# aaletov/open-pcc-metric

Measured on AMD Instinct MI355X. Metric: Mpoints/s for symmetric D1+D2 PSNR, N_ref=N_deg=1M, higher is better.
Workload: dtype f64

## Files before the change

open_pcc_metric_amd/csrc/pccm_api.hip:

```cpp
#include <cxxabi.h>
#include <dlfcn.h>
#include <math.h>
#include <stdarg.h>
#include <stdio.h>
#include <string.h>

#include <chrono>
#include <new>
#include <thread>

#include "pccm_stale.h"

namespace pccm {

static thread_local char g_err[512] = "";

int fail(int code, const char *fmt, ...)
{
    va_list ap;
    va_start(ap, fmt);
    vsnprintf(g_err, sizeof(g_err), fmt, ap);
    va_end(ap);
    return code;
}

int ensure(pccm_ctx *ctx, DevBuf &b, size_t bytes)
{
    if (bytes <= b.bytes && b.p) return PCCM_OK;
    if (ctx->capturing) {
        ctx->capture_failed = true;
        return fail(PCCM_E_STATE, "a buffer must grow during graph capture: run the same call sequence once before capturing");
    }
    ctx->epoch++;
    if (b.p) {
        PCCM_HIP(hipStreamSynchronize(ctx->stream));
        PCCM_HIP(hipFree(b.p));
        b.p = nullptr;
        b.bytes = 0;
    }
    size_t want = bytes < 256 ? 256 : bytes;
    PCCM_HIP(hipMalloc(&b.p, want));
    b.bytes = want;
    return PCCM_OK;
}

int grow(void **p, size_t &cap, size_t bytes)
{
    if (*p && cap >= bytes) return PCCM_OK;
    if (*p) {
        (void)hipFree(*p);
        *p = nullptr;
        cap = 0;
    }
    PCCM_HIP(hipMalloc(p, bytes ? bytes : 1));
    cap = bytes;
    return PCCM_OK;
}

int check_device_errors(pccm_ctx *ctx)
{
    if (!ctx->host_err) return PCCM_OK;
    const uint32_t e = __atomic_exchange_n(ctx->host_err, 0u, __ATOMIC_RELAXED);
    if (!e) return PCCM_OK;
    results_dropped(ctx);
    return fail(PCCM_E_STATE, "a search kernel reported an inconsistent state (device error word 0x%x: %s%s%s): the results of this search were "
                              "dropped, run it again", e, (e & 1u) ? "the tail launch's wait for its own workgroups ran out; " : "",
                (e & 2u) ? "a voxel brick contradicts its cell start; " : "", (e & kErrMergeTable) ? "the duplicate table overflowed" : "");
}

static hipEvent_t take_event(pccm_ctx *ctx)
{
    if (!ctx->event_pool.empty()) {
        hipEvent_t e = ctx->event_pool.back();
        ctx->event_pool.pop_back();
        return e;
    }
    hipEvent_t e = nullptr;
    if (hipEventCreate(&e) != hipSuccess) return nullptr;
    return e;
}

ProfScope::ProfScope(pccm_ctx *c, int k) : ctx(c), cls(k)
{
    if (!ctx->prof_on || ctx->capturing) return;
    a = take_event(ctx);
    b = take_event(ctx);
    if (a) (void)hipEventRecord(a, ctx->stream);
}

ProfScope::~ProfScope()
{
    if (!ctx->prof_on || ctx->capturing || !a || !b) return;
    (void)hipEventRecord(b, ctx->stream);
    ctx->spans.push_back({a, b, cls});
}

static int collect_spans(pccm_ctx *ctx)
{
    if (ctx->spans.empty()) return PCCM_OK;
    PCCM_HIP(hipStreamSynchronize(ctx->stream));
    for (auto &s : ctx->spans) {
        float ms = 0.f;
        if (hipEventElapsedTime(&ms, s.a, s.b) == hipSuccess) {
            ctx->prof_ms[s.cls] += ms;
            ctx->prof_n[s.cls] += 1;
        }
        ctx->event_pool.push_back(s.a);
        ctx->event_pool.push_back(s.b);
    }
    ctx->spans.clear();
    return PCCM_OK;
}

static void free_buf(DevBuf &b)
{
    if (b.p) (void)hipFree(b.p);
    b.p = nullptr;
    b.bytes = 0;
}

// ... 9 lines not shown
}

static void free_nn(NNResult &r)
{
    free_buf(r.flagged);
    free_buf(r.flag_thr);
    free_buf(r.tail);
    free_buf(r.rec);
    r.form = NNForm{};
    if (r.idx) (void)hipFree(r.idx);
    if (r.d2) (void)hipFree(r.d2);
    r.idx = nullptr;
    r.d2 = nullptr;
    r.cap = 0;
}

static void shard_of(int64_t n, int rank, int world, int64_t *b, int64_t *e)
{
    if (world <= 0) {
        *b = 0;
        *e = 0;
        return;
    }
    const int64_t unit = n >= (int64_t)world * kChunk ? kChunk : kLeaf;
    const int64_t units = (n + unit - 1) / unit;
    int64_t u0 = units * rank / world, u1 = units * (rank + 1) / world;
    int64_t lo = u0 * unit, hi = u1 * unit;
    *b = lo < n ? lo : n;
    *e = hi < n ? hi : n;
}

static int dir_clouds(pccm_ctx *ctx, int dir, const Cloud **it, const Cloud **se)
{
    if (dir == PCCM_DIR_LEFT) { *it = &ctx->cloud[0]; *se = &ctx->cloud[1]; }
    else if (dir == PCCM_DIR_RIGHT) { *it = &ctx->cloud[1]; *se = &ctx->cloud[0]; }
    else if (dir == PCCM_DIR_SELF) { *it = &ctx->cloud[0]; *se = &ctx->cloud[0]; }
    else return fail(PCCM_E_ARG, "bad direction %d", dir);
    if ((*it)->n <= 0 || (*se)->n <= 0) return fail(PCCM_E_STATE, "clouds are not set");
    return PCCM_OK;
}

static void host_copy(void *dst, const void *src, size_t bytes)
{
    constexpr size_t kPiece = 1u << 20;
    const int nt = bytes >= 8 * kPiece ? 4 : bytes >= 2 * kPiece ? 2 : 1;
    if (nt == 1) {
        memcpy(dst, src, bytes);
        return;
    }
    std::thread th[3];
    const size_t part = (bytes / nt + 63) & ~(size_t)63;
    for (int k = 1; k < nt; ++k) {
        const size_t off = (size_t)k * part, len = k + 1 < nt ? part : bytes - off;
        th[k - 1] = std::thread([=] { memcpy((char *)dst + off, (const char *)src + off, len); });
    }
    memcpy(dst, src, part);
    for (int k = 1; k < nt; ++k) th[k - 1].join();
}

static int pin_ensure(pccm_ctx *ctx, int which, size_t bytes)
{
    if (ctx->pin_cap[which] >= bytes) return PCCM_OK;
    if (ctx->pin[which]) {
        PCCM_HIP(hipDeviceSynchronize());
        (void)hipHostFree(ctx->pin[which]);
        ctx->pin[which] = nullptr;
        ctx->pin_cap[which] = 0;
    }
    const size_t cap = (bytes + (bytes >> 2) + 4095) & ~(size_t)4095;
    if (hipHostMalloc(&ctx->pin[which], cap, hipHostMallocDefault) != hipSuccess) {
        (void)hipGetLastError();
        ctx->pin[which] = nullptr;
        return fail(PCCM_E_OOM, "hipHostMalloc of %zu bytes (transfer staging) failed", cap);
    }
    ctx->pin_cap[which] = cap;
    return PCCM_OK;
}

constexpr size_t kStagedFrom = 32u << 10;
constexpr size_t kPinWindow = 64u << 20;

static int h2d(pccm_ctx *ctx, void *dev, const void *host, size_t bytes, hipStream_t st)
{
    if (!ctx->io_staged || bytes < kStagedFrom) {
        PCCM_HIP(hipMemcpyAsync(dev, host, bytes, hipMemcpyHostToDevice, st));
        return PCCM_OK;
    }
    const int which = st == ctx->stream ? 0 : 1;
    if (!ctx->pin_ev[which]) PCCM_HIP(hipEventCreateWithFlags(&ctx->pin_ev[which], hipEventDisableTiming));
    if (ctx->pin_ev_set[which]) PCCM_HIP(hipEventSynchronize(ctx->pin_ev[which]));
    int rc = pin_ensure(ctx, which, bytes < kPinWindow ? bytes : kPinWindow);
    if (rc) return rc;
    constexpr size_t kChunk = 4u << 20;
    static_assert(kPinWindow % kChunk == 0, "whole pieces per window");
    for (size_t off = 0; off < bytes; off += kChunk) {
        const size_t len = bytes - off < kChunk ? bytes - off : kChunk, at = off % kPinWindow;
        if (off && at == 0) {
            PCCM_HIP(hipEventRecord(ctx->pin_ev[which], st));
            PCCM_HIP(hipEventSynchronize(ctx->pin_ev[which]));
        }
        host_copy((char *)ctx->pin[which] + at, (const char *)host + off, len);
        PCCM_HIP(hipMemcpyAsync((char *)dev + off, (char *)ctx->pin[which] + at, len, hipMemcpyHostToDevice, st));
    }
    PCCM_HIP(hipEventRecord(ctx->pin_ev[which], st));
    ctx->pin_ev_set[which] = true;
    return PCCM_OK;
}

static int d2h(pccm_ctx *ctx, void *host, const void *dev, size_t bytes)
{
// ... 2365 lines not shown
```

open_pcc_metric_amd/csrc/pccm_gridbuild.hip:

```cpp
#include "pccm_grid.h"

namespace pccm {

constexpr int kLbItems = 64;
constexpr int kLbTile = 256 * kLbItems;

int64_t scan_tiles(int64_t m) { return (m + kLbTile - 1) / kLbTile; }

__global__ __launch_bounds__(256) void k_scan_lookback(uint32_t *__restrict__ data, int64_t m, unsigned long long *__restrict__ state,
                                                       int64_t ntiles)
{
    __shared__ uint32_t s_tile, s_prefix, wsum[4];
    const int tid = threadIdx.x, lane = tid & 63, w = tid >> 6;
    if (tid == 0) s_tile = (uint32_t)atomicAdd(&state[ntiles], 1ull);
    __syncthreads();
    const int64_t tile = s_tile;
    const int64_t base = tile * kLbTile + (int64_t)tid * kLbItems;
    uint32_t v[kLbItems], tot = 0;
    if (base + kLbItems <= m) {
#pragma unroll
        for (int k = 0; k < kLbItems; k += 4) {
            const uint4 q = *reinterpret_cast<const uint4 *>(&data[base + k]);
            v[k] = q.x; v[k + 1] = q.y; v[k + 2] = q.z; v[k + 3] = q.w;
        }
    } else {
#pragma unroll
        for (int k = 0; k < kLbItems; ++k) v[k] = (base + k < m) ? data[base + k] : 0u;
    }
#pragma unroll
    for (int k = 0; k < kLbItems; ++k) tot += v[k];
    uint32_t inc = tot;
#pragma unroll
    for (int off = 1; off < 64; off <<= 1) {
        const uint32_t o = __shfl_up(inc, off);
        if (lane >= off) inc += o;
    }
    if (lane == 63) wsum[w] = inc;
    __syncthreads();
    uint32_t woff = 0;
    for (int k = 0; k < w; ++k) woff += wsum[k];
    const uint32_t agg = wsum[0] + wsum[1] + wsum[2] + wsum[3];
    if (w == 0) {
        if (lane == 0)
            __hip_atomic_store(&state[tile], ((tile == 0 ? 2ull : 1ull) << 32) | agg, __ATOMIC_RELAXED, __HIP_MEMORY_SCOPE_AGENT);
        uint32_t excl = 0;
        int64_t p = tile - 1;
        while (p >= 0) {
            const int64_t idx = p - lane;
            const unsigned long long st = idx >= 0 ? __hip_atomic_load(&state[idx], __ATOMIC_RELAXED, __HIP_MEMORY_SCOPE_AGENT)
                                                   : (2ull << 32);
            const uint32_t status = (uint32_t)(st >> 32), val = (uint32_t)st;
            const unsigned long long incl = __ballot(status == 2u), empty = __ballot(status == 0u);
            const int first = incl ? __ffsll((long long)incl) - 1 : 64;
            const unsigned long long nearer = first >= 64 ? ~0ull : ((1ull << first) - 1ull);
            if (empty & nearer) {
                __builtin_amdgcn_s_sleep(2);
                continue;
            }
            uint32_t part = (lane <= first) ? val : 0u;
#pragma unroll
            for (int off = 32; off > 0; off >>= 1) part += __shfl_xor(part, off);
            excl += part;
            if (first < 64) break;
            p -= 64;
        }
        if (lane == 0) {
            if (tile > 0) __hip_atomic_store(&state[tile], (2ull << 32) | (unsigned long long)(excl + agg), __ATOMIC_RELAXED,
                                             __HIP_MEMORY_SCOPE_AGENT);
            s_prefix = excl;
        }
    }
    __syncthreads();
    uint32_t run = s_prefix + woff + inc - tot;
    if (base + kLbItems <= m) {
#pragma unroll
        for (int k = 0; k < kLbItems; k += 4) {
            uint4 q;
            q.x = run; run += v[k];
            q.y = run; run += v[k + 1];
            q.z = run; run += v[k + 2];
            q.w = run; run += v[k + 3];
            *reinterpret_cast<uint4 *>(&data[base + k]) = q;
        }
    } else {
#pragma unroll
        for (int k = 0; k < kLbItems; ++k) {
            if (base + k < m) data[base + k] = run;
            run += v[k];
        }
    }
}

constexpr int kRegK = 8;
constexpr int kRegRecs = 256 * kRegK;
constexpr int kMaxLg = 13;

struct BinJob {
    const double *x64;
    const float *x32;
    int64_t row0, n;
    uint32_t *cs;
    int64_t tl;
    int64_t nt;
    int64_t hoff;
    int64_t base;
    int64_t tile0;
    const float4 *sp;
    uint32_t *occ;
};

__device__ __forceinline__ void write_cell_starts(const BinJob &J, const uint32_t *s_cnt, int64_t c0, int nc, uint32_t first, uint32_t m)
{
    const int tid = threadIdx.x, nth = (int)blockDim.x;
    if (!J.occ) {
        for (int c = tid; c < nc; c += nth) J.cs[c0 + c] = first + s_cnt[c];
        return;
    }
    for (int c = tid; c < ((nc + 63) & ~63); c += nth) {
        const uint32_t here = c < nc ? s_cnt[c] : m, next = c + 1 < nc ? s_cnt[c + 1] : m;
        if (c < nc) J.cs[c0 + c] = first + here;
        const unsigned long long bits = __ballot(next != here);
        if ((tid & 63) == 0) {
            J.occ[(c0 + c) >> 5] = (uint32_t)bits;
            J.occ[((c0 + c) >> 5) + 1] = (uint32_t)(bits >> 32);
        }
    }
}

struct BinPlan {
    BinJob j[2];
    int njobs;
    int lg;
    int nbin;
    int64_t ncells;
    int64_t ntiles;
    int64_t hlen;
    int64_t state_off;
    int64_t nstate;
    uint32_t *zero;
    int nzero;
    uint32_t *cursor, *toff, *bstart;
};

template <bool X32>
__device__ __forceinline__ void load_point(const BinJob &J, int64_t i, double &x, double &y, double &z)
{
    const int64_t r = J.row0 + i;
    if (X32) {
        const float *q = J.x32 + (r >> 2) * 12 + (r & 3);
        x = (double)q[0];
        y = (double)q[4];
        z = (double)q[8];
    } else {
        const double *p = J.x64 + 3 * r;
        x = p[0];
        y = p[1];
        z = p[2];
    }
}

__device__ __forceinline__ void load_quad(const BinJob &J, int64_t i, float4 &x, float4 &y, float4 &z)
{
    const float4 *q = reinterpret_cast<const float4 *>(J.x32 + ((J.row0 + i) >> 2) * 12);
    x = q[0];
    y = q[1];
    z = q[2];
}

__device__ __forceinline__ int tile_job(const BinPlan &P, int64_t &tile)
{
    if (P.njobs > 1 && tile >= P.j[0].nt) {
        tile -= P.j[0].nt;
        return 1;
    }
    return 0;
}

template <bool X32, bool CUR>
__global__ __launch_bounds__(1024) void k_bin_count(BinPlan P, GridGeom g, uint32_t *__restrict__ hist)
{
    extern __shared__ uint32_t s_hist[];
    const int tid = threadIdx.x, nth = (int)blockDim.x;
    if (!CUR && blockIdx.x == 0) {
        unsigned long long *state = reinterpret_cast<unsigned long long *>(hist + P.state_off);
        if (tid == 0) hist[P.hlen] = 0u;
        for (int64_t k = tid; k < P.nstate; k += nth) state[k] = 0ull;
    }
    for (int b = tid; b < P.nbin; b += nth) s_hist[b] = 0u;
    __syncthreads();
    int64_t tile = blockIdx.x;
    const int jb = tile_job(P, tile);
    const BinJob &J = P.j[jb];
    const int64_t i0 = tile * J.tl, i1 = (i0 + J.tl < J.n) ? i0 + J.tl : J.n;
    if (X32 && J.sp) {
// ... 16 lines not shown
            for (int u = 0; u < 2; ++u) {
                const int64_t q = qd + (int64_t)u * nth;
                load_quad(J, i0 + 4 * (q < nquad ? q : nquad - 1), x[u], y[u], z[u]);
            }
#pragma unroll
            for (int u = 0; u < 2; ++u) {
                const int64_t i = i0 + 4 * (qd + (int64_t)u * nth);
                const float xs[4] = {x[u].x, x[u].y, x[u].z, x[u].w}, ys[4] = {y[u].x, y[u].y, y[u].z, y[u].w},
                            zs[4] = {z[u].x, z[u].y, z[u].z, z[u].w};
#pragma unroll
                for (int k = 0; k < 4; ++k)
                    if (i + k < i1) atomicAdd(&s_hist[cell_linear(g, (double)xs[k], (double)ys[k], (double)zs[k]) >> P.lg], 1u);
            }
        }
    } else {
        for (int64_t i = i0 + tid; i < i1; i += 4 * nth) {
            uint32_t bin[4];
#pragma unroll
            for (int k = 0; k < 4; ++k) {
                const int64_t ii = i + nth * k;
                double x, y, z;
                load_point<X32>(J, ii < i1 ? ii : i1 - 1, x, y, z);
                bin[k] = cell_linear(g, x, y, z) >> P.lg;
            }
#pragma unroll
            for (int k = 0; k < 4; ++k)
                if (i + nth * k < i1) atomicAdd(&s_hist[bin[k]], 1u);
        }
    }
    __syncthreads();
    if (CUR) {
        uint32_t *cur = P.cursor + (int64_t)jb * P.nbin, *dst = P.toff + (J.tile0 + tile) * P.nbin;
        for (int b = tid; b < P.nbin; b += nth) {
            const uint32_t c = s_hist[b];
            dst[b] = c ? atomicAdd(&cur[b], c) : 0u;
        }
        return;
    }
    uint32_t *dst = hist + J.hoff + tile;
    for (int b = tid; b < P.nbin; b += nth) dst[(int64_t)b * J.nt] = s_hist[b];
}

__device__ __forceinline__ void block_scan_inplace(uint32_t *s_cnt, int nc, uint32_t *s_wsum, uint32_t *s_carry);

template <typename REC, bool X32, bool CUR>
__global__ __launch_bounds__(1024) void k_bin_scatter(BinPlan P, GridGeom g, const uint32_t *__restrict__ hist, REC *__restrict__ tmp)
{
    extern __shared__ uint32_t s_cur[];
    __shared__ uint32_t s_wsum[16], s_carry;
    const int tid = threadIdx.x, nth = (int)blockDim.x;
    int64_t tile = blockIdx.x;
    const int jb = tile_job(P, tile);
    const BinJob &J = P.j[jb];
    if (CUR) {
        const uint32_t *tot = P.cursor + (int64_t)jb * P.nbin, *off = P.toff + (J.tile0 + tile) * P.nbin;
        uint32_t mine[2];
#pragma unroll
        for (int k = 0; k < 2; ++k) mine[k] = (tid + nth * k < P.nbin) ? off[tid + nth * k] : 0u;
        for (int b = tid; b < P.nbin; b += nth) s_cur[b] = tot[b];
        __syncthreads();
        block_scan_inplace(s_cur, P.nbin, s_wsum, &s_carry);
        if (tile == 0) {
            uint32_t *bs = P.bstart + (int64_t)jb * P.nbin;
            for (int b = tid; b < P.nbin; b += nth) bs[b] = (uint32_t)J.base + s_cur[b];
        }
        if (blockIdx.x == 0) {
            const BinJob &L = P.j[P.njobs - 1];
            if (tid == 0) P.bstart[(int64_t)P.njobs * P.nbin] = (uint32_t)(L.base + L.n);
            for (int k = 0; k < P.njobs; ++k)
                if (P.j[k].nt == 0)
                    for (int b = tid; b < P.nbin; b += nth) P.bstart[(int64_t)k * P.nbin + b] = (uint32_t)P.j[k].base;
        }
        __syncthreads();
#pragma unroll
        for (int k = 0; k < 2; ++k)
            if (tid + nth * k < P.nbin) s_cur[tid + nth * k] += (uint32_t)J.base + mine[k];
        for (int b = tid + 2 * nth; b < P.nbin; b += nth) s_cur[b] += (uint32_t)J.base + off[b];
    } else {
        const uint32_t *src = hist + J.hoff + tile;
        for (int b = tid; b < P.nbin; b += nth) s_cur[b] = src[(int64_t)b * J.nt];
    }
    __syncthreads();
    const int64_t i0 = tile * J.tl, i1 = (i0 + J.tl < J.n) ? i0 + J.tl : J.n;
    if (X32 && J.sp) {
        float4 *__restrict__ out = reinterpret_cast<float4 *>(tmp);
        for (int64_t i = i0 + tid; i < i1; i += 8 * nth) {
            float4 r[8];
#pragma unroll
            for (int k = 0; k < 8; ++k) {
                const int64_t ii = i + (int64_t)nth * k;
                r[k] = J.sp[J.row0 + (ii < i1 ? ii : i1 - 1)];
            }
#pragma unroll
            for (int k = 0; k < 8; ++k)
                if (i + (int64_t)nth * k < i1) {
                    const uint32_t pos = atomicAdd(&s_cur[cell_linear(g, (double)r[k].x, (double)r[k].y, (double)r[k].z) >> P.lg], 1u);
                    if (sizeof(REC) == 16) out[pos] = r[k];
                }
        }
        return;
    }
    if (X32) {
        const int64_t nquad = (i1 - i0 + 3) >> 2;
        for (int64_t qd = tid; qd < nquad; qd += 2 * nth) {
            float4 x[2], y[2], z[2];
#pragma unroll
// ... 39 lines not shown
}

__device__ __forceinline__ void block_scan_inplace(uint32_t *s_cnt, int nc, uint32_t *s_wsum, uint32_t *s_carry)
{
    const int tid = threadIdx.x, lane = tid & 63, w = tid >> 6;
    if (tid == 0) *s_carry = 0u;
    __syncthreads();
    const int nth = (int)blockDim.x;
    for (int base = 0; base < nc; base += 4 * nth) {
        const int e = base + 4 * tid;
        uint32_t c0 = e < nc ? s_cnt[e] : 0u, c1 = e + 1 < nc ? s_cnt[e + 1] : 0u;
        uint32_t c2 = e + 2 < nc ? s_cnt[e + 2] : 0u, c3 = e + 3 < nc ? s_cnt[e + 3] : 0u;
        const uint32_t tot = c0 + c1 + c2 + c3;
        uint32_t inc = tot;
#pragma unroll
        for (int off = 1; off < 64; off <<= 1) {
            const uint32_t o = __shfl_up(inc, off);
            if (lane >= off) inc += o;
        }
        if (lane == 63) s_wsum[w] = inc;
        __syncthreads();
        uint32_t run = *s_carry + inc - tot;
        for (int k = 0; k < w; ++k) run += s_wsum[k];
        if (e < nc) s_cnt[e] = run;
        run += c0;
        if (e + 1 < nc) s_cnt[e + 1] = run;
        run += c1;
        if (e + 2 < nc) s_cnt[e + 2] = run;
        run += c2;
        if (e + 3 < nc) s_cnt[e + 3] = run;
        __syncthreads();
        if (tid == nth - 1) *s_carry = run + c3;
        __syncthreads();
    }
}

__device__ __forceinline__ uint32_t rec_cell(const GridGeom &g, const float4 &r) { return cell_linear(g, (double)r.x, (double)r.y, (double)r.z); }
__device__ __forceinline__ uint32_t rec_cell(const GridGeom &g, const double4 &r) { return cell_linear(g, r.x, r.y, r.z); }
template <typename REC> struct RawRec;
template <> struct RawRec<Rec32> { typedef float4 type; };
template <> struct RawRec<GridRec> { typedef double4 type; };

template <typename REC>
__global__ __launch_bounds__(256, sizeof(REC) == 16 ? 6 : 4) void k_bin_sort(BinPlan P, GridGeom g, const uint32_t *__restrict__ hist, const REC *__restrict__ tmp,
                                                  REC *__restrict__ recs)
{
    extern __shared__ uint32_t s_cnt[];
    __shared__ uint32_t s_wsum[16], s_carry;
    const int tid = threadIdx.x;
    const int jb = (P.njobs > 1 && (int)blockIdx.x >= P.nbin) ? 1 : 0;
    const int b = (int)blockIdx.x - jb * P.nbin;
    const BinJob &J = P.j[jb];
    uint32_t s, e, j0;
    if (P.cursor) {
        const uint32_t *bs = P.bstart + (int64_t)jb * P.nbin + b;
        s = bs[0];
        e = bs[1];
        j0 = (uint32_t)J.base;
        if (tid == 0) P.cursor[(int64_t)jb * P.nbin + b] = 0u;
    } else {
        s = hist[J.hoff + (int64_t)b * J.nt];
        e = hist[J.hoff + (int64_t)(b + 1) * J.nt];
        j0 = hist[J.hoff];
    }
    const uint32_t m = e - s;
    const int64_t c0 = (int64_t)b << P.lg;
    const int nc = (int)((c0 + (1ll << P.lg) < P.ncells ? c0 + (1ll << P.lg) : P.ncells) - c0);
    for (int c = tid; c < nc; c += 256) s_cnt[c] = 0u;
    __syncthreads();
    if (m <= (uint32_t)kRegRecs) {
        typedef typename RawRec<REC>::type RAW;
        const RAW *__restrict__ src = reinterpret_cast<const RAW *>(tmp);
        RAW *__restrict__ dst = reinterpret_cast<RAW *>(recs);
        RAW v[kRegK];
        uint32_t cell[kRegK], rank[kRegK];
#pragma unroll
        for (int k = 0; k < kRegK; ++k) {
            const uint32_t i = tid + 256u * k;
            if (i < m) v[k] = src[s + i];
        }
#pragma unroll
        for (int k = 0; k < kRegK; ++k)
            if (tid + 256u * k < m) {
                cell[k] = rec_cell(g, v[k]) - (uint32_t)c0;
                rank[k] = atomicAdd(&s_cnt[cell[k]], 1u);
            }
        __syncthreads();
        block_scan_inplace(s_cnt, nc, s_wsum, &s_carry);
        write_cell_starts(J, s_cnt, c0, nc, s - j0, m);
#pragma unroll
        for (int k = 0; k < kRegK; ++k)
            if (tid + 256u * k < m) dst[s + s_cnt[cell[k]] + rank[k]] = v[k];
    } else {
        for (uint32_t i = tid; i < m; i += 256) {
            const P3 v = load_rec(tmp, s + i);
            atomicAdd(&s_cnt[cell_linear(g, v.x, v.y, v.z) - (uint32_t)c0], 1u);
        }
        __syncthreads();
        block_scan_inplace(s_cnt, nc, s_wsum, &s_carry);
        write_cell_starts(J, s_cnt, c0, nc, s - j0, m);
        __syncthreads();
        for (uint32_t i = tid; i < m; i += 256) {
            const P3 v = load_rec(tmp, s + i);
            const uint32_t pos = atomicAdd(&s_cnt[cell_linear(g, v.x, v.y, v.z) - (uint32_t)c0], 1u);
            store_rec(recs, s + pos, v);
        }
    }
    if (b == P.nbin - 1 && tid == 0) J.cs[P.ncells] = e - j0;
    if (blockIdx.x == 0 && tid < P.nzero) P.zero[tid] = 0u;
}

static int ceil_log2(int64_t v)
{
    int l = 0;
    while ((1ll << l) < v) ++l;
    return l;
}

int sort_by_cell(pccm_ctx *ctx, const BuildJobs &jobs, const GridGeom &g, int64_t ncells, void *recs, bool rec32, uint32_t *zero, int nzero)
{
    BinPlan P;
    P.zero = zero;
    P.nzero = zero ? nzero : 0;
    P.njobs = jobs.njobs;
    P.ncells = ncells;
    int lg = ceil_log2((ncells + 8191) / 8192);
    P.lg = lg < 10 ? 10 : (lg > kMaxLg ? kMaxLg : lg);
    {
        int64_t nmax = 0;
        for (int k = 0; k < jobs.njobs; ++k) nmax = jobs.j[k].n > nmax ? jobs.j[k].n : nmax;
        while (P.lg > 6 && (double)nmax * (double)(1ll << P.lg) / (double)ncells > 2000.0 && ((ncells >> (P.lg - 1)) + 1) <= 8192) --P.lg;
    }
    static const int lg_env = [] { const char *e = PCCM_DIAG_ENV("PCCM_BUILD_LG"); return e ? atoi(e) : 0; }();
    if (lg_env >= 8 && lg_env <= kMaxLg && (ncells >> lg_env) < 8192) P.lg = lg_env;
    P.nbin = (int)((ncells + (1ll << P.lg) - 1) >> P.lg);
    if (P.nbin > 8192) return fail(PCCM_E_ARG, "grid of %lld cells is too large", (long long)ncells);
    P.ntiles = 0;
    for (int k = 0; k < 2; ++k) {
        const BuildJob &s = jobs.j[k < jobs.njobs ? k : 0];
        BinJob &d = P.j[k];
        d.x64 = s.x64; d.x32 = s.x32; d.row0 = s.row0; d.cs = s.cs;
        d.sp = rec32 ? reinterpret_cast<const float4 *>(s.sp) : nullptr;
        d.occ = s.occ;
        if (rec32 && k < jobs.njobs && (s.row0 & 3)) return fail(PCCM_E_ARG, "a shard must start on a multiple of 4 rows (it starts on 128-row units)");
        d.n = k < jobs.njobs ? s.n : 0;
        static const int64_t tile_rows = [] { const char *e = getenv("PCCM_BUILD_TILE"); int64_t v = e ? atoll(e) : 8192; return v >= 256 ? v : 8192; }();
        int64_t nt = (d.n + tile_rows - 1) / tile_rows;
        if (nt > 1024) nt = 1024;
        d.nt = nt;
        d.tl = nt > 0 ? ((d.n + nt - 1) / nt + 255) / 256 * 256 : 256;
        if (nt > 0) d.nt = (d.n + d.tl - 1) / d.tl;
        d.hoff = (int64_t)P.nbin * P.ntiles;
        d.tile0 = P.ntiles;
        d.base = k == 0 ? 0 : P.j[0].n;
        if (k < jobs.njobs) P.ntiles += d.nt;
    }
    P.hlen = (int64_t)P.nbin * P.ntiles;
    const int64_t st = scan_tiles(P.hlen + 1);
    P.nstate = st + 1;
    P.state_off = (P.hlen + 2) / 2 * 2;
    const size_t rsz = rec32 ? sizeof(Rec32) : sizeof(GridRec);
    static const int bin_threads = [] { const char *e = getenv("PCCM_BUILD_THREADS"); int v = e ? atoi(e) : 1024; return (v >= 64 && v <= 1024 && v % 64 == 0) ? v : 1024; }();
    static const bool use_scan = [] { const char *e = getenv("PCCM_BUILD_SCAN"); return e && e[0] == '1'; }();
    const bool cur = !use_scan && P.nbin <= 8192;
    const int64_t ncur = (int64_t)P.njobs * P.nbin;
    const size_t cur_words = (size_t)(2 * 8192 + 2 * 8192 + 2);
    const size_t hist_bytes = cur ? (cur_words + (size_t)P.hlen) * sizeof(uint32_t)
                                  : (size_t)P.state_off * sizeof(uint32_t) + (size_t)P.nstate * 8;
    int rc;
    const size_t bins_before = ctx->g_bins.bytes;
    if ((rc = ensure(ctx, ctx->g_bins, hist_bytes > cur_words * sizeof(uint32_t) ? hist_bytes : cur_words * sizeof(uint32_t)))) return rc;
    if ((rc = ensure(ctx, ctx->g_tmp, (size_t)(jobs.total > 0 ? jobs.total : 1) * rsz))) return rc;
    uint32_t *hist = (uint32_t *)ctx->g_bins.p;
    P.cursor = P.toff = P.bstart = nullptr;
    if (cur) {
        P.cursor = hist;
        P.bstart = hist + 2 * 8192;
        P.toff = hist + cur_words;
        if (ctx->g_bins.bytes != bins_before || !ctx->bins_clean) {
            if (ctx->capturing) {
                ctx->capture_failed = true;
                return fail(PCCM_E_STATE, "the grid build's scratch must exist before graph capture: run the sequence once first");
            }
            PCCM_HIP(hipMemsetAsync(hist, 0, (size_t)2 * 8192 * sizeof(uint32_t), ctx->stream));
        }
        ctx->bins_clean = false;
    }
    unsigned long long *state = reinterpret_cast<unsigned long long *>(hist + P.state_off);
    const size_t lds_bins = (size_t)P.nbin * sizeof(uint32_t), lds_cells = ((size_t)1 << P.lg) * sizeof(uint32_t);
    if (P.ntiles > 0 && cur) {
        dim3 tg((unsigned)P.ntiles);
        if (rec32) PCCM_LAUNCH(ctx, (k_bin_count<true, true>), tg, dim3(bin_threads), lds_bins, ctx->stream, P, g, hist);
        else PCCM_LAUNCH(ctx, (k_bin_count<false, true>), tg, dim3(bin_threads), lds_bins, ctx->stream, P, g, hist);
        if (rec32) PCCM_LAUNCH(ctx, (k_bin_scatter<Rec32, true, true>), tg, dim3(bin_threads), lds_bins, ctx->stream, P, g, (const uint32_t *)hist, (Rec32 *)ctx->g_tmp.p);
        else PCCM_LAUNCH(ctx, (k_bin_scatter<GridRec, false, true>), tg, dim3(bin_threads), lds_bins, ctx->stream, P, g, (const uint32_t *)hist, (GridRec *)ctx->g_tmp.p);
    } else if (P.ntiles > 0) {
        dim3 tg((unsigned)P.ntiles);
        if (rec32) PCCM_LAUNCH(ctx, (k_bin_count<true, false>), tg, dim3(bin_threads), lds_bins, ctx->stream, P, g, hist);
        else PCCM_LAUNCH(ctx, (k_bin_count<false, false>), tg, dim3(bin_threads), lds_bins, ctx->stream, P, g, hist);
        PCCM_LAUNCH(ctx, k_scan_lookback, dim3((unsigned)st), dim3(256), 0, ctx->stream, hist, P.hlen + 1, state, st);
        if (rec32) PCCM_LAUNCH(ctx, (k_bin_scatter<Rec32, true, false>), tg, dim3(bin_threads), lds_bins, ctx->stream, P, g, (const uint32_t *)hist, (Rec32 *)ctx->g_tmp.p);
        else PCCM_LAUNCH(ctx, (k_bin_scatter<GridRec, false, false>), tg, dim3(bin_threads), lds_bins, ctx->stream, P, g, (const uint32_t *)hist, (GridRec *)ctx->g_tmp.p);
    } else if (cur) {
        PCCM_HIP(hipMemsetAsync(P.bstart, 0, (size_t)(ncur + 1) * sizeof(uint32_t), ctx->stream));
    } else {
        PCCM_HIP(hipMemsetAsync(hist, 0, hist_bytes, ctx->stream));
    }
    dim3 bg((unsigned)(P.nbin * P.njobs));
    if (rec32) PCCM_LAUNCH(ctx, (k_bin_sort<Rec32>), bg, dim3(256), lds_cells, ctx->stream, P, g, (const uint32_t *)hist, (const Rec32 *)ctx->g_tmp.p, (Rec32 *)recs);
    else PCCM_LAUNCH(ctx, (k_bin_sort<GridRec>), bg, dim3(256), lds_cells, ctx->stream, P, g, (const uint32_t *)hist, (const GridRec *)ctx->g_tmp.p, (GridRec *)recs);
    PCCM_HIP(hipGetLastError());
    ctx->bins_clean = true;
    return PCCM_OK;
}

}
```

open_pcc_metric_amd/csrc/pccm_internal.h:

```cpp
#pragma once
#include <hip/hip_runtime.h>
#include <stdint.h>
#include <mutex>
#include <string>
#include <vector>

#include "pccm.h"

#ifdef PCCM_DIAG
#define PCCM_DIAG_ENV(name) getenv(name)
#else
#define PCCM_DIAG_ENV(name) (static_cast<const char *>(nullptr))
#endif

namespace pccm {

constexpr int kScanThreads = 256;
constexpr int kScanTile = 1024;
constexpr int kTileVec = kScanTile / 4 * 3;
constexpr int kGranule = 64;
constexpr float kBig32 = 3.0e38f;
constexpr float kPadCoord = 1.0e18f;
constexpr double kMaxAbsCoord = 1.0e15;

// ... 415 lines not shown
{
#pragma unroll
    for (int off = 1; off < 64; off <<= 1) {
        const uint32_t o = __shfl_up(v, off);
        if (lane >= off) v += o;
    }
    return v;
}

__device__ __forceinline__ double angular_similarity(const double *a, const double *b)
{
    const double dot = __dadd_rn(__dadd_rn(__dmul_rn(a[0], b[0]), __dmul_rn(a[1], b[1])), __dmul_rn(a[2], b[2]));
    const double na2 = __dadd_rn(__dadd_rn(__dmul_rn(a[0], a[0]), __dmul_rn(a[1], a[1])), __dmul_rn(a[2], a[2]));
    const double nb2 = __dadd_rn(__dadd_rn(__dmul_rn(b[0], b[0]), __dmul_rn(b[1], b[1])), __dmul_rn(b[2], b[2]));
    const double den = __dsqrt_rn(__dmul_rn(na2, nb2));
    if (den == 0.0) return 0.0;
    const double q = __ddiv_rn(fabs(dot), den);
    const double c = q > 1.0 ? 1.0 : q;
    return __dsub_rn(1.0, __ddiv_rn(__dmul_rn(2.0, acos(c)), M_PI));
}

__device__ __forceinline__ double ssim_similarity(double a, double b)
{
    const double num = fabs(__dsub_rn(a, b));
    const double den = __dadd_rn(fmax(fabs(a), fabs(b)), 0x1.0p-52);
    return __dsub_rn(1.0, __ddiv_rn(num, den));
}

__host__ __device__ __forceinline__ bool is_p2d_metric(int metric)
{
    return metric >= PCCM_METRIC_P2D && metric <= PCCM_METRIC_P2D_JOINT;
}

__host__ __device__ __forceinline__ bool is_stored_metric(int metric)
{
    return is_p2d_metric(metric) || metric == PCCM_METRIC_RESOLUTION;
}

__host__ __device__ __forceinline__ bool is_ssim_metric(int metric)
{
    return metric >= PCCM_METRIC_SSIM_GEOMETRY && metric <= PCCM_METRIC_SSIM_COLOR;
}

struct PointJob {
    const double *q64, *r64, *nrm;
    const double *c64, *cn64;
    const double *inrm;
    const float4 *recs;
    const int32_t *idx;
    int64_t q_begin;
    int metric, normal_mode;
    double *val;
};
constexpr uint32_t kErrMergeTable = 4u;
struct MergeLayout {
    int64_t nw, nsw;
    uint64_t cap;
    size_t doubles;
    size_t bits, rep, wpre, spre, table, words;
    size_t bytes() const { return doubles * sizeof(double) + words * sizeof(uint32_t); }
};
__host__ __device__ inline MergeLayout merge_layout(int64_t n)
{
    MergeLayout L;
    L.nw = (n + 63) / 64;
    L.nsw = (L.nw + 63) / 64;
    L.cap = 64;
    while (L.cap < 2 * (uint64_t)n) L.cap <<= 1;
    L.doubles = (size_t)12 * (size_t)n;
    L.bits = 4;
    L.rep = L.bits + 2 * (size_t)L.nw;
    L.wpre = L.rep + (size_t)n;
    L.spre = L.wpre + (size_t)L.nw;
    L.table = L.spre + (size_t)L.nsw;
    L.words = L.table + (size_t)L.cap;
    return L;
}
struct PointJobs {
    PointJob j[4];
    int njobs;
    int64_t off[5];
};
constexpr int kSelBits = 11, kSelBins = 1 << kSelBits;
constexpr int kSelPasses = 6;
constexpr int kSelMax = 8;
constexpr int kSelPerCol = 4;
constexpr size_t kSelLds = (size_t)kSelPerCol * kSelBins * sizeof(uint32_t) + 256;
struct SelState {
    unsigned long long prefix;
    unsigned long long k;
};
struct UnitSelect {
    int pass = 0;
    int nsel = 0;
    int sfirst[9] = {};
    int boff[9] = {};
    unsigned long long k[kSelMax] = {};
    double *out[kSelMax] = {};
    uint32_t *hist = nullptr;
    SelState *state = nullptr;
};
struct UnitJobs {
    UnitJob j[8];
    int njobs;
    int64_t uoff[9];
    int64_t toff[9];
// ... 37 lines not shown
```

Before: 10620.

## Fuse bin count and scatter into one pass with per-tile piece lists

When records are 32-bit and all jobs have staged float4 points, the grid build now runs one scatter kernel instead of count, scan and scatter. Each tile bins its rows locally, publishes per-bin totals and piece descriptors through global atomics, and writes its rows into tile-local order. The per-bin sort kernel then reassembles each bin from these pieces by binary search, and it clears the double-buffered totals for the next call using an epoch flag. This drops a kernel launch and a pass over the input, at the cost of non-contiguous gather reads, extra atomics and new consistency checks reported through an error word.

```diff
diff --git a/open_pcc_metric_amd/csrc/pccm_api.hip b/open_pcc_metric_amd/csrc/pccm_api.hip
--- a/open_pcc_metric_amd/csrc/pccm_api.hip
+++ b/open_pcc_metric_amd/csrc/pccm_api.hip
@@ -7,6 +7,7 @@
 
 #include <chrono>
 #include <new>
+#include <system_error>
 #include <thread>
 
 #include "pccm_stale.h"
@@ -63,9 +64,10 @@
     const uint32_t e = __atomic_exchange_n(ctx->host_err, 0u, __ATOMIC_RELAXED);
     if (!e) return PCCM_OK;
     results_dropped(ctx);
-    return fail(PCCM_E_STATE, "a search kernel reported an inconsistent state (device error word 0x%x: %s%s%s): the results of this search were "
+    return fail(PCCM_E_STATE, "a search kernel reported an inconsistent state (device error word 0x%x: %s%s%s%s): the results of this search were "
                               "dropped, run it again", e, (e & 1u) ? "the tail launch's wait for its own workgroups ran out; " : "",
-                (e & 2u) ? "a voxel brick contradicts its cell start; " : "", (e & kErrMergeTable) ? "the duplicate table overflowed" : "");
+                (e & 2u) ? "a voxel brick contradicts its cell start; " : "", (e & kErrMergeTable) ? "the duplicate table overflowed; " : "",
+                (e & kErrBinState) ? "the grid build's bin totals contradict its plan" : "");
 }
 
 static hipEvent_t take_event(pccm_ctx *ctx)
@@ -181,10 +183,15 @@
     const size_t part = (bytes / nt + 63) & ~(size_t)63;
     for (int k = 1; k < nt; ++k) {
         const size_t off = (size_t)k * part, len = k + 1 < nt ? part : bytes - off;
-        th[k - 1] = std::thread([=] { memcpy((char *)dst + off, (const char *)src + off, len); });
+        try {
+            th[k - 1] = std::thread([=] { memcpy((char *)dst + off, (const char *)src + off, len); });
+        } catch (const std::system_error &) {
+            memcpy((char *)dst + off, (const char *)src + off, len);
+        }
     }
     memcpy(dst, src, part);
-    for (int k = 1; k < nt; ++k) th[k - 1].join();
+    for (int k = 1; k < nt; ++k)
+        if (th[k - 1].joinable()) th[k - 1].join();
 }
 
 static int pin_ensure(pccm_ctx *ctx, int which, size_t bytes)
diff --git a/open_pcc_metric_amd/csrc/pccm_binplan.h b/open_pcc_metric_amd/csrc/pccm_binplan.h
--- /dev/null
+++ b/open_pcc_metric_amd/csrc/pccm_binplan.h
@@ -0,0 +1,110 @@
+#pragma once
+#include <cstddef>
+#include <cstdint>
+
+namespace pccm {
+
+constexpr int kBinMax = 8192;
+constexpr int kMaxLg = 13;
+constexpr int kGrpBins = 64;
+constexpr int kGrpMax = kBinMax / kGrpBins;
+constexpr int kScatterRegRows = 8;
+constexpr int64_t kMaxTiles = 1024;
+
+constexpr int64_t kBinCursorOff = 0;
+constexpr int64_t kBinBstartOff = kBinCursorOff + 2 * kBinMax;
+constexpr int64_t kBinFineOff = kBinBstartOff + 2 * kBinMax + 2;
+constexpr int64_t kBinCoarseOff = kBinFineOff + 2 * (2 * 2 * (int64_t)kBinMax);
+constexpr int64_t kBinEpochOff = kBinCoarseOff + 2 * 2 * kGrpMax;
+constexpr int64_t kBinFixedWords = kBinEpochOff + 2;
+static_assert(kBinFineOff % 2 == 0 && kBinFixedWords % 2 == 0, "64-bit words behind the fixed part stay aligned");
+
+struct BinKnobs {
+    int64_t tile_rows = 8192;
+    int threads = 1024;
+    int lg = 0;
+    bool scan = false;
+    bool pieces = true;
+};
+
+struct BinJobShape {
+    int64_t n;
+    int64_t tl;
+    int64_t nt;
+    int64_t hoff;
+    int64_t base;
+    int64_t tile0;
+};
+
+struct BinShape {
+    int njobs, lg, nbin, ngrp;
+    int64_t ncells, ntiles, hlen;
+    int64_t state_off, nstate, nscan;
+    bool cur;
+    bool pieces;
+    bool one_pass;
+    int64_t max_nt;
+    int64_t var_off, var_words;
+    size_t bytes;
+    BinJobShape j[2];
+};
+
+inline int binplan_ceil_log2(int64_t v)
+{
+    int l = 0;
+    while ((1ll << l) < v) ++l;
+    return l;
+}
+
+constexpr int64_t kBinScanTile = 256 * 64;
+
+inline int bin_plan(BinShape &S, int njobs, const int64_t n[2], const bool sp[2], int64_t ncells, bool rec32, const BinKnobs &K)
+{
+    S.njobs = njobs;
+    S.ncells = ncells;
+    int lg = binplan_ceil_log2((ncells + kBinMax - 1) / kBinMax);
+    lg = lg < 10 ? 10 : (lg > kMaxLg ? kMaxLg : lg);
+    int64_t nmax = 0;
+    for (int k = 0; k < njobs; ++k) nmax = n[k] > nmax ? n[k] : nmax;
+    while (lg > 6 && (double)nmax * (double)(1ll << lg) / (double)ncells > 2000.0 && ((ncells >> (lg - 1)) + 1) <= kBinMax) --lg;
+    if (K.lg >= 8 && K.lg <= kMaxLg && (ncells >> K.lg) < kBinMax) lg = K.lg;
+    S.lg = lg;
+    const int64_t nbin = (ncells + (1ll << lg) - 1) >> lg;
+    S.nbin = (int)nbin;
+    S.ngrp = (int)((nbin + kGrpBins - 1) / kGrpBins);
+    if (nbin > kBinMax) return -1;
+    S.ntiles = 0;
+    S.max_nt = 0;
+    bool all_sp = njobs > 0, one_pass = true;
+    for (int k = 0; k < 2; ++k) {
+        BinJobShape &d = S.j[k];
+        d.n = k < njobs ? n[k] : 0;
+        int64_t nt = (d.n + K.tile_rows - 1) / K.tile_rows;
+        if (nt > kMaxTiles) nt = kMaxTiles;
+        d.nt = nt;
+        d.tl = nt > 0 ? ((d.n + nt - 1) / nt + 255) / 256 * 256 : 256;
+        if (nt > 0) d.nt = (d.n + d.tl - 1) / d.tl;
+        d.hoff = nbin * S.ntiles;
+        d.tile0 = S.ntiles;
+        d.base = k == 0 ? 0 : S.j[0].n;
+        if (k < njobs) {
+            S.ntiles += d.nt;
+            S.max_nt = d.nt > S.max_nt ? d.nt : S.max_nt;
+            all_sp = all_sp && sp[k];
+            one_pass = one_pass && d.tl <= (int64_t)kScatterRegRows * K.threads;
+        }
+    }
+    S.hlen = nbin * S.ntiles;
+    S.nscan = (S.hlen + 1 + kBinScanTile - 1) / kBinScanTile;
+    S.nstate = S.nscan + 1;
+    S.state_off = (S.hlen + 2) / 2 * 2;
+    S.cur = !K.scan;
+    S.pieces = S.cur && K.pieces && rec32 && all_sp && S.ntiles > 0;
+    S.one_pass = S.pieces && one_pass;
+    S.var_off = kBinFixedWords;
+    S.var_words = (S.cur && K.pieces && rec32) ? 2 * S.hlen : S.hlen;
+    S.bytes = S.cur ? (size_t)(S.var_off + S.var_words) * sizeof(uint32_t) : (size_t)S.state_off * sizeof(uint32_t) + (size_t)S.nstate * 8;
+    return 0;
+}
+
+}
diff --git a/open_pcc_metric_amd/csrc/pccm_gridbuild.hip b/open_pcc_metric_amd/csrc/pccm_gridbuild.hip
--- a/open_pcc_metric_amd/csrc/pccm_gridbuild.hip
+++ b/open_pcc_metric_amd/csrc/pccm_gridbuild.hip
@@ -1,4 +1,5 @@
 #include "pccm_grid.h"
+#include "pccm_binplan.h"
 
 namespace pccm {
 
@@ -93,7 +94,6 @@
 
 constexpr int kRegK = 8;
 constexpr int kRegRecs = 256 * kRegK;
-constexpr int kMaxLg = 13;
 
 struct BinJob {
     const double *x64;
@@ -140,6 +140,11 @@
     uint32_t *zero;
     int nzero;
     uint32_t *cursor, *toff, *bstart;
+    int pieces, max_nt;
+    unsigned long long *fine;
+    uint32_t *coarse, *epoch;
+    uint2 *plist;
+    uint32_t *err;
 };
 
 template <bool X32>
@@ -262,6 +267,101 @@
     int64_t tile = blockIdx.x;
     const int jb = tile_job(P, tile);
     const BinJob &J = P.j[jb];
+    if (CUR && X32 && sizeof(REC) == 16 && P.pieces) {
+        const int lane = tid & 63;
+        const uint32_t sel = P.epoch[0] & 1u;
+        if (blockIdx.x == 0 && tid == 0) P.epoch[1] = sel;
+        for (int b = tid; b < P.nbin; b += nth) s_cur[b] = 0u;
+        __syncthreads();
+        const int64_t i0 = tile * J.tl, i1 = (i0 + J.tl < J.n) ? i0 + J.tl : J.n;
+        const uint32_t rows = (uint32_t)(i1 - i0), first = (uint32_t)(J.base + i0);
+        const bool one_pass = J.tl <= (int64_t)kScatterRegRows * nth;
+        float4 *__restrict__ out = reinterpret_cast<float4 *>(tmp);
+        float4 r[kScatterRegRows];
+        uint32_t bin[kScatterRegRows], rank[kScatterRegRows];
+        if (one_pass) {
+#pragma unroll
+            for (int k = 0; k < kScatterRegRows; ++k) {
+                const int64_t ii = i0 + tid + (int64_t)nth * k;
+                r[k] = J.sp[J.row0 + (ii < i1 ? ii : i1 - 1)];
+            }
+#pragma unroll
+            for (int k = 0; k < kScatterRegRows; ++k)
+                if (i0 + tid + (int64_t)nth * k < i1) {
+                    bin[k] = cell_linear(g, (double)r[k].x, (double)r[k].y, (double)r[k].z) >> P.lg;
+                    rank[k] = atomicAdd(&s_cur[bin[k]], 1u);
+                }
+        } else {
+            for (int64_t i = i0 + tid; i < i1; i += (int64_t)kScatterRegRows * nth) {
+                float4 q[kScatterRegRows];
+#pragma unroll
+                for (int k = 0; k < kScatterRegRows; ++k) {
+                    const int64_t ii = i + (int64_t)nth * k;
+                    q[k] = J.sp[J.row0 + (ii < i1 ? ii : i1 - 1)];
+                }
+#pragma unroll
+                for (int k = 0; k < kScatterRegRows; ++k)
+                    if (i + (int64_t)nth * k < i1) atomicAdd(&s_cur[cell_linear(g, (double)q[k].x, (double)q[k].y, (double)q[k].z) >> P.lg], 1u);
+            }
+        }
+        __syncthreads();
+        unsigned long long *fine = P.fine + ((int64_t)sel * 2 + jb) * kBinMax;
+        uint32_t *coarse = P.coarse + ((int64_t)sel * 2 + jb) * kGrpMax;
+        uint2 *list = P.plist + J.hoff;
+        const uint32_t c0 = tid < P.nbin ? s_cur[tid] : 0u;
+        unsigned long long old0 = 0ull;
+        if (c0) old0 = atomicAdd(&fine[tid], (1ull << 32) | (unsigned long long)c0);
+        {
+            uint32_t gs = c0;
+#pragma unroll
+            for (int o = 32; o > 0; o >>= 1) gs += __shfl_xor(gs, o);
+            if (lane == 0 && gs) atomicAdd(&coarse[tid >> 6], gs);
+        }
+        block_scan_inplace(s_cur, P.nbin, s_wsum, &s_carry);
+        if (one_pass) {
+#pragma unroll
+            for (int k = 0; k < kScatterRegRows; ++k)
+                if (i0 + tid + (int64_t)nth * k < i1) out[first + s_cur[bin[k]] + rank[k]] = r[k];
+        }
+        for (int b0 = 0; b0 < P.nbin; b0 += nth) {
+            const int b = b0 + tid;
+            uint32_t off = 0u, c = 0u;
+            if (b < P.nbin) {
+                off = s_cur[b];
+                c = (b + 1 < P.nbin ? s_cur[b + 1] : rows) - off;
+            }
+            unsigned long long old = old0;
+            if (b0 > 0) {
+                if (c) old = atomicAdd(&fine[b], (1ull << 32) | (unsigned long long)c);
+                uint32_t gs = c;
+#pragma unroll
+                for (int o = 32; o > 0; o >>= 1) gs += __shfl_xor(gs, o);
+                if (lane == 0 && gs) atomicAdd(&coarse[b >> 6], gs);
+            }
+            if (c) {
+                const uint32_t slot = (uint32_t)(old >> 32);
+                if (slot < (uint32_t)J.nt) list[(int64_t)b * J.nt + slot] = make_uint2(first + off, c);
+                else if (P.err) atomicOr(P.err, kErrBinState);
+            }
+        }
+        if (one_pass) return;
+        __syncthreads();
+        for (int64_t i = i0 + tid; i < i1; i += (int64_t)kScatterRegRows * nth) {
+            float4 q[kScatterRegRows];
+#pragma unroll
+            for (int k = 0; k < kScatterRegRows; ++k) {
+                const int64_t ii = i + (int64_t)nth * k;
+                q[k] = J.sp[J.row0 + (ii < i1 ? ii : i1 - 1)];
+            }
+#pragma unroll
+            for (int k = 0; k < kScatterRegRows; ++k)
+                if (i + (int64_t)nth * k < i1) {
+                    const uint32_t pos = atomicAdd(&s_cur[cell_linear(g, (double)q[k].x, (double)q[k].y, (double)q[k].z) >> P.lg], 1u);
+                    out[first + pos] = q[k];
+                }
+        }
+        return;
+    }
     if (CUR) {
         const uint32_t *tot = P.cursor + (int64_t)jb * P.nbin, *off = P.toff + (J.tile0 + tile) * P.nbin;
         uint32_t mine[2];
@@ -407,7 +507,86 @@
     const int b = (int)blockIdx.x - jb * P.nbin;
     const BinJob &J = P.j[jb];
     uint32_t s, e, j0;
-    if (P.cursor) {
+    uint32_t np = 0u;
+    uint32_t *s_ps = s_cnt + ((size_t)1 << P.lg), *s_po = s_ps + P.max_nt + 1;
+    const bool pieces = sizeof(REC) == 16 && P.pieces;
+    if (pieces) {
+        const int lane = tid & 63, w = tid >> 6, grp = b >> 6;
+        const uint32_t sel = P.epoch[1] & 1u;
+        const unsigned long long *fine = P.fine + ((int64_t)sel * 2 + jb) * kBinMax;
+        const uint32_t *coarse = P.coarse + ((int64_t)sel * 2 + jb) * kGrpMax;
+        const uint2 *list = P.plist + J.hoff + (int64_t)b * J.nt;
+        const uint2 mine = tid < J.nt ? list[tid] : make_uint2(0u, 0u);
+        uint32_t part = 0u;
+        if (tid < grp) part = coarse[tid];
+        else if (tid >= 128 && tid < 192 && grp * 64 + (tid - 128) < b) part = (uint32_t)fine[grp * 64 + (tid - 128)];
+        const unsigned long long tot = fine[b];
+        np = (uint32_t)(tot >> 32);
+        uint32_t mrec = (uint32_t)tot;
+        const uint32_t lim = (uint32_t)(P.j[1].base + P.j[1].n);
+        bool bad = np > (uint32_t)J.nt;
+        if (bad) np = 0u;
+        const bool small = J.nt <= 256;
+        uint32_t len = 0u;
+        if (small && tid < np) {
+            if (mine.x > lim || mine.y > lim - mine.x) bad = true;
+            else len = mine.y;
+        }
+        uint32_t inc = len;
+#pragma unroll
+        for (int o = 1; o < 64; o <<= 1) {
+            const uint32_t up = __shfl_up(inc, o);
+            if (lane >= o) inc += up;
+        }
+#pragma unroll
+        for (int o = 32; o > 0; o >>= 1) part += __shfl_xor(part, o);
+        if (lane == 0) s_wsum[w] = part;
+        if (lane == 63) s_wsum[4 + w] = inc;
+        {
+            unsigned long long *other = P.fine + (int64_t)(sel ^ 1u) * 2 * kBinMax;
+            const int per = (2 * kBinMax + (int)gridDim.x - 1) / (int)gridDim.x;
+            const int z0 = (int)blockIdx.x * per, z1 = z0 + per < 2 * kBinMax ? z0 + per : 2 * kBinMax;
+            for (int z = z0 + tid; z < z1; z += 256) other[z] = 0ull;
+            if (blockIdx.x == 0) {
+                P.coarse[(int64_t)(sel ^ 1u) * 2 * kGrpMax + tid] = 0u;
+                if (tid == 0) P.epoch[0] = sel ^ 1u;
+            }
+        }
+        __syncthreads();
+        j0 = (uint32_t)J.base;
+        s = j0 + s_wsum[0] + s_wsum[1] + s_wsum[2] + s_wsum[3];
+        if (small) {
+            uint32_t woff = 0u;
+            for (int k = 0; k < w; ++k) woff += s_wsum[4 + k];
+            if (tid < np) {
+                s_ps[tid] = woff + inc - len;
+                s_po[tid] = mine.x;
+            }
+            if (s_wsum[4] + s_wsum[5] + s_wsum[6] + s_wsum[7] != mrec) bad = true;
+        } else {
+            for (uint32_t p = tid; p < np; p += 256) {
+                uint2 d = p < 256u ? mine : list[p];
+                if (d.x > lim || d.y > lim - d.x) {
+                    bad = true;
+                    d.y = 0u;
+                }
+                s_ps[p] = d.y;
+                s_po[p] = d.x;
+            }
+            __syncthreads();
+            block_scan_inplace(s_ps, (int)np, s_wsum, &s_carry);
+            if (s_carry != mrec) bad = true;
+        }
+        if (s - j0 > (uint32_t)J.n || mrec > (uint32_t)J.n - (s - j0)) bad = true;
+        if (__syncthreads_or(bad)) {
+            if (tid == 0 && P.err) atomicOr(P.err, kErrBinState);
+            if (s - j0 > (uint32_t)J.n) s = j0;
+            np = 0u;
+            mrec = 0u;
+        }
+        e = s + mrec;
+        if (tid == 0) s_ps[np] = mrec;
+    } else if (P.cursor) {
         const uint32_t *bs = P.bstart + (int64_t)jb * P.nbin + b;
         s = bs[0];
         e = bs[1];
@@ -429,10 +608,26 @@
         RAW *__restrict__ dst = reinterpret_cast<RAW *>(recs);
         RAW v[kRegK];
         uint32_t cell[kRegK], rank[kRegK];
-#pragma unroll
-        for (int k = 0; k < kRegK; ++k) {
-            const uint32_t i = tid + 256u * k;
-            if (i < m) v[k] = src[s + i];
+        if (pieces) {
+#pragma unroll
+            for (int k = 0; k < kRegK; ++k) {
+                const uint32_t i = tid + 256u * k;
+                if (i < m) {
+                    uint32_t lo = 0u, hi = np;
+                    while (hi - lo > 1u) {
+                        const uint32_t mid = (lo + hi) >> 1;
+                        if (s_ps[mid] <= i) lo = mid;
+                        else hi = mid;
+                    }
+                    v[k] = src[s_po[lo] + (i - s_ps[lo])];
+                }
+            }
+        } else {
+#pragma unroll
+            for (int k = 0; k < kRegK; ++k) {
+                const uint32_t i = tid + 256u * k;
+                if (i < m) v[k] = src[s + i];
+            }
         }
 #pragma unroll
         for (int k = 0; k < kRegK; ++k)
@@ -446,6 +641,26 @@
 #pragma unroll
         for (int k = 0; k < kRegK; ++k)
             if (tid + 256u * k < m) dst[s + s_cnt[cell[k]] + rank[k]] = v[k];
+    } else if (pieces) {
+        for (uint32_t p = 0; p < np; ++p) {
+            const uint32_t o = s_po[p], len = s_ps[p + 1] - s_ps[p];
+            for (uint32_t i = tid; i < len; i += 256) {
+                const P3 v = load_rec(tmp, o + i);
+                atomicAdd(&s_cnt[cell_linear(g, v.x, v.y, v.z) - (uint32_t)c0], 1u);
+            }
+        }
+        __syncthreads();
+        block_scan_inplace(s_cnt, nc, s_wsum, &s_carry);
+        write_cell_starts(J, s_cnt, c0, nc, s - j0, m);
+        __syncthreads();
+        for (uint32_t p = 0; p < np; ++p) {
+            const uint32_t o = s_po[p], len = s_ps[p + 1] - s_ps[p];
+            for (uint32_t i = tid; i < len; i += 256) {
+                const P3 v = load_rec(tmp, o + i);
+                const uint32_t pos = atomicAdd(&s_cnt[cell_linear(g, v.x, v.y, v.z) - (uint32_t)c0], 1u);
+                store_rec(recs, s + pos, v);
+            }
+        }
     } else {
         for (uint32_t i = tid; i < m; i += 256) {
             const P3 v = load_rec(tmp, s + i);
@@ -465,85 +680,100 @@
     if (blockIdx.x == 0 && tid < P.nzero) P.zero[tid] = 0u;
 }
 
-static int ceil_log2(int64_t v)
-{
-    int l = 0;
-    while ((1ll << l) < v) ++l;
-    return l;
+static_assert(2 * kGrpMax == 256 && kGrpBins == 64, "k_bin_sort clears the coarse totals with one workgroup; a wave of k_bin_scatter covers a group");
+static_assert(kBinScanTile == kLbTile, "pccm_binplan.h sizes the look-back scan's state");
+
+static const BinKnobs &bin_knobs()
+{
+    static const BinKnobs K = [] {
+        BinKnobs k;
+        const char *e = getenv("PCCM_BUILD_TILE");
+        const int64_t t = e ? atoll(e) : 8192;
+        k.tile_rows = t >= 256 ? t : 8192;
+        e = getenv("PCCM_BUILD_THREADS");
+        const int v = e ? atoi(e) : 1024;
+        k.threads = (v >= 64 && v <= 1024 && v % 64 == 0) ? v : 1024;
+        e = PCCM_DIAG_ENV("PCCM_BUILD_LG");
+        k.lg = e ? atoi(e) : 0;
+        e = getenv("PCCM_BUILD_SCAN");
+        k.scan = e && e[0] == '1';
+        e = getenv("PCCM_BUILD_PIECES");
+        k.pieces = !(e && e[0] == '0');
+        return k;
+    }();
+    return K;
 }
 
 int sort_by_cell(pccm_ctx *ctx, const BuildJobs &jobs, const GridGeom &g, int64_t ncells, void *recs, bool rec32, uint32_t *zero, int nzero)
 {
+    const BinKnobs &K = bin_knobs();
+    BinShape S;
+    int64_t n[2] = {0, 0};
+    bool sp[2] = {false, false};
+    for (int k = 0; k < jobs.njobs; ++k) {
+        n[k] = jobs.j[k].n;
+        sp[k] = rec32 && jobs.j[k].sp;
+        if (rec32 && (jobs.j[k].row0 & 3)) return fail(PCCM_E_ARG, "a shard must start on a multiple of 4 rows (it starts on 128-row units)");
+    }
+    if (bin_plan(S, jobs.njobs, n, sp, ncells, rec32, K)) return fail(PCCM_E_ARG, "grid of %lld cells is too large", (long long)ncells);
     BinPlan P;
     P.zero = zero;
     P.nzero = zero ? nzero : 0;
-    P.njobs = jobs.njobs;
+    P.njobs = S.njobs;
     P.ncells = ncells;
-    int lg = ceil_log2((ncells + 8191) / 8192);
-    P.lg = lg < 10 ? 10 : (lg > kMaxLg ? kMaxLg : lg);
-    {
-        int64_t nmax = 0;
-        for (int k = 0; k < jobs.njobs; ++k) nmax = jobs.j[k].n > nmax ? jobs.j[k].n : nmax;
-        while (P.lg > 6 && (double)nmax * (double)(1ll << P.lg) / (double)ncells > 2000.0 && ((ncells >> (P.lg - 1)) + 1) <= 8192) --P.lg;
-    }
-    static const int lg_env = [] { const char *e = PCCM_DIAG_ENV("PCCM_BUILD_LG"); return e ? atoi(e) : 0; }();
-    if (lg_env >= 8 && lg_env <= kMaxLg && (ncells >> lg_env) < 8192) P.lg = lg_env;
-    P.nbin = (int)((ncells + (1ll << P.lg) - 1) >> P.lg);
-    if (P.nbin > 8192) return fail(PCCM_E_ARG, "grid of %lld cells is too large", (long long)ncells);
-    P.ntiles = 0;
+    P.lg = S.lg;
+    P.nbin = S.nbin;
+    P.ntiles = S.ntiles;
+    P.hlen = S.hlen;
+    P.nstate = S.nstate;
+    P.state_off = S.state_off;
+    P.pieces = S.pieces ? 1 : 0;
+    P.max_nt = S.pieces ? (int)S.max_nt : 0;
     for (int k = 0; k < 2; ++k) {
         const BuildJob &s = jobs.j[k < jobs.njobs ? k : 0];
         BinJob &d = P.j[k];
         d.x64 = s.x64; d.x32 = s.x32; d.row0 = s.row0; d.cs = s.cs;
         d.sp = rec32 ? reinterpret_cast<const float4 *>(s.sp) : nullptr;
         d.occ = s.occ;
-        if (rec32 && k < jobs.njobs && (s.row0 & 3)) return fail(PCCM_E_ARG, "a shard must start on a multiple of 4 rows (it starts on 128-row units)");
-        d.n = k < jobs.njobs ? s.n : 0;
-        static const int64_t tile_rows = [] { const char *e = getenv("PCCM_BUILD_TILE"); int64_t v = e ? atoll(e) : 8192; return v >= 256 ? v : 8192; }();
-        int64_t nt = (d.n + tile_rows - 1) / tile_rows;
-        if (nt > 1024) nt = 1024;
-        d.nt = nt;
-        d.tl = nt > 0 ? ((d.n + nt - 1) / nt + 255) / 256 * 256 : 256;
-        if (nt > 0) d.nt = (d.n + d.tl - 1) / d.tl;
-        d.hoff = (int64_t)P.nbin * P.ntiles;
-        d.tile0 = P.ntiles;
-        d.base = k == 0 ? 0 : P.j[0].n;
-        if (k < jobs.njobs) P.ntiles += d.nt;
-    }
-    P.hlen = (int64_t)P.nbin * P.ntiles;
-    const int64_t st = scan_tiles(P.hlen + 1);
-    P.nstate = st + 1;
-    P.state_off = (P.hlen + 2) / 2 * 2;
+        d.n = S.j[k].n; d.tl = S.j[k].tl; d.nt = S.j[k].nt; d.hoff = S.j[k].hoff; d.tile0 = S.j[k].tile0; d.base = S.j[k].base;
+    }
+    const int64_t st = S.nscan;
     const size_t rsz = rec32 ? sizeof(Rec32) : sizeof(GridRec);
-    static const int bin_threads = [] { const char *e = getenv("PCCM_BUILD_THREADS"); int v = e ? atoi(e) : 1024; return (v >= 64 && v <= 1024 && v % 64 == 0) ? v : 1024; }();
-    static const bool use_scan = [] { const char *e = getenv("PCCM_BUILD_SCAN"); return e && e[0] == '1'; }();
-    const bool cur = !use_scan && P.nbin <= 8192;
+    const bool cur = S.cur;
     const int64_t ncur = (int64_t)P.njobs * P.nbin;
-    const size_t cur_words = (size_t)(2 * 8192 + 2 * 8192 + 2);
-    const size_t hist_bytes = cur ? (cur_words + (size_t)P.hlen) * sizeof(uint32_t)
-                                  : (size_t)P.state_off * sizeof(uint32_t) + (size_t)P.nstate * 8;
     int rc;
     const size_t bins_before = ctx->g_bins.bytes;
-    if ((rc = ensure(ctx, ctx->g_bins, hist_bytes > cur_words * sizeof(uint32_t) ? hist_bytes : cur_words * sizeof(uint32_t)))) return rc;
+    if ((rc = ensure(ctx, ctx->g_bins, S.bytes > (size_t)kBinFixedWords * sizeof(uint32_t) ? S.bytes : (size_t)kBinFixedWords * sizeof(uint32_t)))) return rc;
     if ((rc = ensure(ctx, ctx->g_tmp, (size_t)(jobs.total > 0 ? jobs.total : 1) * rsz))) return rc;
     uint32_t *hist = (uint32_t *)ctx->g_bins.p;
-    P.cursor = P.toff = P.bstart = nullptr;
+    P.cursor = P.toff = P.bstart = P.coarse = P.epoch = nullptr;
+    P.fine = nullptr;
+    P.plist = nullptr;
+    P.err = ctx->host_err;
     if (cur) {
-        P.cursor = hist;
-        P.bstart = hist + 2 * 8192;
-        P.toff = hist + cur_words;
+        P.cursor = hist + kBinCursorOff;
+        P.bstart = hist + kBinBstartOff;
+        P.fine = reinterpret_cast<unsigned long long *>(hist + kBinFineOff);
+        P.coarse = hist + kBinCoarseOff;
+        P.epoch = hist + kBinEpochOff;
+        P.toff = hist + S.var_off;
+        P.plist = reinterpret_cast<uint2 *>(hist + S.var_off);
         if (ctx->g_bins.bytes != bins_before || !ctx->bins_clean) {
             if (ctx->capturing) {
                 ctx->capture_failed = true;
                 return fail(PCCM_E_STATE, "the grid build's scratch must exist before graph capture: run the sequence once first");
             }
-            PCCM_HIP(hipMemsetAsync(hist, 0, (size_t)2 * 8192 * sizeof(uint32_t), ctx->stream));
+            PCCM_HIP(hipMemsetAsync(hist, 0, (size_t)kBinFixedWords * sizeof(uint32_t), ctx->stream));
         }
         ctx->bins_clean = false;
     }
     unsigned long long *state = reinterpret_cast<unsigned long long *>(hist + P.state_off);
-    const size_t lds_bins = (size_t)P.nbin * sizeof(uint32_t), lds_cells = ((size_t)1 << P.lg) * sizeof(uint32_t);
-    if (P.ntiles > 0 && cur) {
+    const int bin_threads = K.threads;
+    const size_t lds_bins = (size_t)P.nbin * sizeof(uint32_t);
+    const size_t lds_cells = (((size_t)1 << P.lg) + (S.pieces ? 2 * (size_t)S.max_nt + 1 : 0)) * sizeof(uint32_t);
+    if (S.pieces) {
+        PCCM_LAUNCH(ctx, (k_bin_scatter<Rec32, true, true>), dim3((unsigned)P.ntiles), dim3(bin_threads), lds_bins, ctx->stream, P, g, (const uint32_t *)hist, (Rec32 *)ctx->g_tmp.p);
+    } else if (P.ntiles > 0 && cur) {
         dim3 tg((unsigned)P.ntiles);
         if (rec32) PCCM_LAUNCH(ctx, (k_bin_count<true, true>), tg, dim3(bin_threads), lds_bins, ctx->stream, P, g, hist);
         else PCCM_LAUNCH(ctx, (k_bin_count<false, true>), tg, dim3(bin_threads), lds_bins, ctx->stream, P, g, hist);
@@ -559,7 +789,7 @@
     } else if (cur) {
         PCCM_HIP(hipMemsetAsync(P.bstart, 0, (size_t)(ncur + 1) * sizeof(uint32_t), ctx->stream));
     } else {
-        PCCM_HIP(hipMemsetAsync(hist, 0, hist_bytes, ctx->stream));
+        PCCM_HIP(hipMemsetAsync(hist, 0, S.bytes, ctx->stream));
     }
     dim3 bg((unsigned)(P.nbin * P.njobs));
     if (rec32) PCCM_LAUNCH(ctx, (k_bin_sort<Rec32>), bg, dim3(256), lds_cells, ctx->stream, P, g, (const uint32_t *)hist, (const Rec32 *)ctx->g_tmp.p, (Rec32 *)recs);
diff --git a/open_pcc_metric_amd/csrc/pccm_internal.h b/open_pcc_metric_amd/csrc/pccm_internal.h
--- a/open_pcc_metric_amd/csrc/pccm_internal.h
+++ b/open_pcc_metric_amd/csrc/pccm_internal.h
@@ -491,6 +491,7 @@
     int metric, normal_mode;
     double *val;
 };
+constexpr uint32_t kErrBinState = 8u;
 constexpr uint32_t kErrMergeTable = 4u;
 struct MergeLayout {
     int64_t nw, nsw;
```

Measured after the change: 10380. 2.3% lower.
